# teshnizi/GraphEnvs

Measured on AMD Instinct MI355X. Metric: env-steps/sec (whole node), ShortestPath-v0 n=64 m=192 batch=65536, 1/2/4/8 GPU, higher is better.
Workload: dtype u64; 1 GPU; ShortestPath-v0 n_nodes=64 n_edges=192 weighted, 65536 env slots per GPU, random valid actions on device, same-step autoreset (seed-exact G(n,m)+features on device); envs_per_gpu=65536, prefetch_period=0, episodes_finished_per_gpu=6165512, settle_steps=128, parallelism=batch shard x1, no collective

## Files before the change

### graphenvs_amd/csrc/ge_api.hip

```cpp
#include <math.h>
#include <stdio.h>
#include <stdlib.h>
#include <string.h>

#include <initializer_list>
#include <memory>
#include <new>
#include <vector>

#include "ge_params.h"
#include "ge_platform.h"
#include "ge_reset.h"
#include "ge_features.h"
#include "ge_step.h"
#include "ge_tsp_eval.h"
#include "ge_spare.h"

#define GE_MAX_BUCKETS 4
struct GeBucket {
  bool used;
  bool list_only;
  struct { int lds, pre, grid; } graph;
  struct { int lds, pre_off, threads, grid; } gen;
};
struct GePlan {
  int n_buckets;
  GeBucket bk[GE_MAX_BUCKETS];
  int nseed;
  bool feat_fast;
  int f64_lds, f64_pre_off, feat_grid;
  GeLds inject;
};
static int bucket_of(int n) { return n <= 128 ? 0 : (n <= 256 ? 1 : (n <= 512 ? 2 : 3)); }
static bool takes_generic(const GeParams &C) { return C.n > 64 || C.spatial; }

typedef void (*GeBaselineFn)(GeParams, GeRagged, int, uint8_t *, uint64_t);
struct GeKernels {
  void (*reset)(GeParams, GeRagged, const uint32_t *, GeRun, GeInject, int, int);
  void (*features)(GeParams, GeRagged, GeRun, int, int);
  void (*features64)(GeParams, GeRagged, GeRun, int);
  void (*feat_combine)(GeParams, GeRagged, GeRun);
  void (*swap)(GeParams, GeRagged, GeRagged, ge_buffers, int);
  void (*sample)(GeParams, GeRagged, uint64_t, int64_t *);
  void (*dc_range)(GeParams, GeRagged, const int64_t *);
  void (*tsp_closure)(GeParams, GeRagged, int, uint8_t *, uint64_t, int);
  GeBaselineFn tsp_tour, mis_baseline, steiner_baseline;
  void (*step[2])(GeParams, GeRagged, const int64_t *, uint64_t);
  int step_threads;
  size_t step_lds;
  bool step_quad;
  void (*step_path64[2][2])(GeParams, const int64_t *, uint64_t);
};

struct ge_engine {
  GeParams P;
  ge_config cfg;
  GeKernels k = {};
  GePlan plan = {};
  hipEvent_t ev[4];
  bool have_events = false;
  int n_classes = 0;
  GeRagged R = {};
  int aw_max;
  std::vector<GeParams> classes;
  bool loaded = false;
  bool seeded = false;
  bool streams = false;
  bool spares = false;
  GeParams PS;
  GeRagged RS = {};
  std::vector<GeParams> classesS;
  int period = 0, swap_parts = 1;
  int64_t pending_calls = 0;
  int32_t *refill_list = nullptr, *refill_count = nullptr;
};

static GeRun run_full() { GeRun r = {GE_ITEMS_ALL, 1, 0, 0, 0, 0, 0}; return r; }
static GeRun run_inject(bool seeds) { GeRun r = {GE_ITEMS_ALL, seeds ? 2 : 0, 0, 0, 1, 0, 0}; return r; }
static GeRun run_continue() { GeRun r = {GE_ITEMS_ALL, 0, 1, 1, 0, 0, 0}; return r; }
static GeRun run_queue(const ge_engine *e) { GeRun r = {GE_ITEMS_QUEUE, 0, 1, 0, 0, 0, e->spares ? 2 : GE_SEED_DEPTH}; return r; }
static GeRun run_refill() { GeRun r = {GE_ITEMS_QUEUE, 0, 1, 0, 0, 1, 2}; return r; }
static GeRun as_list(GeRun r) { r.items = GE_ITEMS_LIST; return r; }


static thread_local char g_err[256] = "";
static int fail(int code, const char *msg) { snprintf(g_err, sizeof(g_err), "%s", msg); return code; }
extern "C" const char *ge_last_error(void) { return g_err; }
extern "C" int ge_abi_version(void) { return GE_ABI_VERSION; }
#ifndef GE_SOURCE_HASH
#define GE_SOURCE_HASH "unknown"
#endif
static const char g_source_hash[] = "GE_SOURCE_HASH=" GE_SOURCE_HASH;
extern "C" const char *ge_source_hash(void) { return g_source_hash + 15; }

static const int kMaxLds = 160 * 1024;
static const GeInject kNoInject = {nullptr, nullptr, nullptr, nullptr, nullptr};
static int step_blocks(int64_t B) { return (int)((B + GE_STEP_BLOCK - 1) / GE_STEP_BLOCK); }
static int prefix_bytes(int64_t B) { return (step_blocks(B) + 2) * 4; }
static bool carves_fit(std::initializer_list<int> bytes) { for (int b : bytes) if (b > kMaxLds) return false; return true; }
static int resident_grid(int lds, int64_t B) {
  int per_cu = kMaxLds / (lds > 0 ? lds : 1);
  if (per_cu > 16) per_cu = 16;
  if (per_cu < 1) per_cu = 1;
  return 256 * per_cu > B ? (int)B : 256 * per_cu;
}
static int64_t obs_len(const GeParams &P) { return (int64_t)P.n * P.F + (int64_t)P.E * P.Fe + 2 * (int64_t)P.E; }
static bool prunes(const GeParams &P) { return (P.env_type == GE_LONGEST_PATH || P.env_type == GE_TSP) && P.parenting >= 2; }
#ifndef GE_NP_EARLY_MAX
#define GE_NP_EARLY_MAX 256
#endif

#define GE_FOR_ENV(env_type, stmt)                                                           \
  do {                                                                                       \
// ... 144 lines not shown
  k.sample = ge_k_sample<RAGGED>;
  k.dc_range = ge_k_dc_range<RAGGED>;
  k.tsp_closure = ge_k_tsp_closure<RAGGED>;
  k.tsp_tour = ge_k_tsp_tour<RAGGED>;
  k.mis_baseline = ge_k_mis_baseline<RAGGED>;
  k.steiner_baseline = ge_k_steiner_baseline<RAGGED>;
  k.step[0] = ge_k_step<ENV, false, RAGGED, 0>; k.step[1] = ge_k_step<ENV, true, RAGGED, 0>;
  k.step_threads = GE_STEP_BLOCK;
  k.step_lds = (size_t)GE_STEP_BLOCK * e->P.W * 8 + GE_STEP_BLOCK + 64;
  if constexpr (ENV == GE_STEINER_TREE || ENV == GE_MULTICAST_ROUTING) {
    if (edge_quad(e)) {
      k.step[0] = ge_k_step_edge<ENV, false, RAGGED>; k.step[1] = ge_k_step_edge<ENV, true, RAGGED>;
      k.step_quad = true;
      k.step_threads = GE_EDGE_THREADS;
      k.step_lds = ge_edge_lds_bytes(e->aw_max, e->P.W) + (RAGGED ? GE_EDGE_CLASS_BYTES : 0);
    }
  }
  if constexpr (ENV == GE_LONGEST_PATH || ENV == GE_TSP) {
    if (prunes(e->P) && e->P.W > GE_MAXW) { k.step[0] = ge_k_step<ENV, false, RAGGED, 2>; k.step[1] = ge_k_step<ENV, true, RAGGED, 2>; }
    else if (prunes(e->P)) { k.step[0] = ge_k_step<ENV, false, RAGGED, 1>; k.step[1] = ge_k_step<ENV, true, RAGGED, 1>; }
  }
  if constexpr (!RAGGED) {
    if (path64(e)) {
      k.step_path64[0][0] = ge_k_step_path64<false, false>; k.step_path64[0][1] = ge_k_step_path64<false, true>;
      k.step_path64[1][0] = ge_k_step_path64<true, false>; k.step_path64[1][1] = ge_k_step_path64<true, true>;
    }
  }
}

static bool raise_lds(const void *kernel, size_t bytes) {
  (void)kernel;
  return bytes <= 64 * 1024 || (hipError_t)GE_SET_MAX_DYN_LDS(kernel, bytes) == hipSuccess;
}

static int finish_create(ge_engine *e) {
  const GeParams &P = e->P;
  const bool rg = e->n_classes > 0;
  const int nblk = step_blocks(P.B), pre2 = prefix_bytes(P.B);
  GE_FOR_ENV(P.env_type, if (rg) (select_kernels<ENV, true>(e)); else (select_kernels<ENV, false>(e)));
  GePlan &L = e->plan;
  auto behind = [&](int body, int &pre) { pre = ge_align16(body); return pre + pre2; };
  const GeParams *first = rg ? e->classes.data() : &e->P;
  const int n_classes = rg ? e->n_classes : 1;
  L.n_buckets = rg ? GE_MAX_BUCKETS : 1;
  int graph_lds = 0, gen_lds = 0;
  int gen_body = 0, f64_body = 0;
  for (int b = 0; b < L.n_buckets; b++) {
    GeBucket &K = L.bk[b];
    int graph = 0, gen = 0, all = 0, waves = 1;
    for (const GeParams *C = first; C < first + n_classes; C++) {
      if (C->bucket != b) continue;
      K.used = true;
      if (C->lds.total > graph) graph = C->lds.total;
      if (C->ldsf.total > all) all = C->ldsf.total;
      if (takes_generic(*C)) { if (C->ldsf.total > gen) gen = C->ldsf.total; if (C->ldsf.waves > waves) waves = C->ldsf.waves; }
      else { L.feat_fast = true; const int body = ge_f64_pre_off(C->E, C->env_type == GE_TSP, nblk); if (body > f64_body) f64_body = body; }
    }
    if (!K.used) continue;
    K.list_only = gen == 0;
    if (gen > gen_body) gen_body = gen;
    K.graph.grid = resident_grid(graph, P.B);
    K.graph.pre = P.lds.pre; K.graph.lds = graph;
    if (rg && P.lds.pre != 0) K.graph.lds = behind(graph, K.graph.pre);
    if (K.graph.lds > graph_lds) graph_lds = K.graph.lds;
    K.gen.threads = GE_WAVE * waves;
    K.gen.pre_off = P.ldsf.pre; K.gen.lds = P.ldsf.total;
    if (rg) K.gen.lds = behind(K.list_only ? all : gen, K.gen.pre_off);
    K.gen.grid = resident_grid(K.gen.lds, P.B);
    if (K.list_only && (rg || K.gen.grid > 8)) K.gen.grid = 8;
    if (K.gen.lds > gen_lds) gen_lds = K.gen.lds;
  }
  if (!rg) L.inject = inject_carve(P, P.B);
  if (!carves_fit({graph_lds, L.inject.total, gen_lds})) return fail(GE_E_TOOBIG, "per-env graph does not fit 160 KiB of LDS");
  L.nseed = (resident_grid(graph_lds, P.B) + 63) / 64;
  if (!raise_lds((const void *)e->k.reset, graph_lds > L.inject.total ? graph_lds : L.inject.total)) return fail(GE_E_LAUNCH, "cannot raise the dynamic LDS limit of the reset kernel");
  if (!raise_lds((const void *)e->k.step[0], e->k.step_lds) || !raise_lds((const void *)e->k.step[1], e->k.step_lds))
    return fail(GE_E_LAUNCH, e->k.step_quad ? "cannot raise the dynamic LDS limit of the edge step kernel" : "cannot raise the dynamic LDS limit of the step kernel");
  L.f64_pre_off = ge_align16(f64_body);
  L.f64_lds = L.feat_fast ? L.f64_pre_off + GE_F64_ITEMS * 4 * 4 + 16 : 0;
  if (!carves_fit({L.f64_lds})) return fail(GE_E_TOOBIG, "feature kernel does not fit LDS");
  if (!raise_lds((const void *)e->k.features, gen_lds)) return fail(GE_E_LAUNCH, "cannot raise the dynamic LDS limit of the feature kernel");
  if (L.feat_fast && !raise_lds((const void *)e->k.features64, L.f64_lds)) return fail(GE_E_LAUNCH, "cannot raise the dynamic LDS limit of the n<=64 feature kernel");
  L.feat_grid = resident_grid(L.feat_fast ? L.f64_lds : gen_body, P.B);
  return GE_OK;
}

extern "C" int ge_create(const ge_config *cfg, const ge_buffers *bufs, ge_engine **out) {
  if (!bufs || !out) return fail(GE_E_BADARG, "null argument");
  GeParams P;
  int rc = derive(cfg, P);
  if (rc != GE_OK) return rc;
  rc = check_buffers(P, bufs);
  if (rc != GE_OK) return rc;
  P.buf = *bufs;
  std::unique_ptr<ge_engine> e(new (std::nothrow) ge_engine());
  if (!e) return fail(GE_E_BADARG, "out of host memory");
  e->P = P; e->cfg = *cfg; e->aw_max = P.AW;
  rc = finish_create(e.get());
  if (rc == GE_OK) *out = e.release();
  return rc;
}

extern "C" int64_t ge_ragged_table_bytes(int32_t n_classes) { return (int64_t)sizeof(GeParams) * (n_classes > 0 ? n_classes : 0); }

extern "C" int ge_create_ragged(const ge_config *cfgs, const ge_buffers *bufs, int32_t n_classes, void *class_table,
                                int32_t *slot_class, int32_t *class_start, ge_engine **out) {
  if (!cfgs || !bufs || !out || !class_table || !slot_class || !class_start || n_classes < 1) return fail(GE_E_BADARG, "null argument");
  const int t = cfgs[0].env_type;
  int64_t total = 0;
  for (int c = 0; c < n_classes; c++) total += cfgs[c].num_envs;
  if (total > 8192 * GE_STEP_BLOCK) return fail(GE_E_TOOBIG, "num_envs > 2M per engine");
  std::unique_ptr<ge_engine> e(new (std::nothrow) ge_engine());
  if (!e) return fail(GE_E_BADARG, "out of host memory");
  e->classes.resize(n_classes);
  std::vector<int32_t> start(n_classes + 1, 0), cls_of((size_t)total);
  int widest = 0, aw_max = 0;
  for (int c = 0; c < n_classes; c++) {
    GeParams &C = e->classes[c];
    int rc = derive(&cfgs[c], C, (int)total);
    if (rc == GE_OK) rc = check_buffers(C, &bufs[c]);
    if (rc == GE_OK && (cfgs[c].env_type != t || cfgs[c].autoreset != cfgs[0].autoreset || cfgs[c].seed_stride != cfgs[0].seed_stride))
      rc = fail(GE_E_BADARG, "the classes of a multi-class engine share env_type, autoreset and seed_stride");
    if (rc == GE_OK && (cfgs[c].weighted != cfgs[0].weighted || cfgs[c].parenting != cfgs[0].parenting || cfgs[c].spatial != cfgs[0].spatial ||
                        cfgs[c].is_eval_env != cfgs[0].is_eval_env))
      rc = fail(GE_E_BADARG, "the classes of a multi-class engine share weighted, parenting, spatial and is_eval_env (they differ in n, m and the per-instance scalars only)");
    if (rc == GE_OK && (cfgs[c].env_index_base != cfgs[0].env_index_base + start[c] || bufs[c].seed != bufs[0].seed + start[c] ||
                        bufs[c].episode != bufs[0].episode + start[c] || bufs[c].mt_state != bufs[0].mt_state + (int64_t)start[c] * GE_SEED_DEPTH * 2 * GE_MT_N))
      rc = fail(GE_E_BADARG, "classes follow one another in slot order: env_index_base, seed, episode and mt_state of class c start at its first global slot");
    if (rc == GE_OK && (bufs[c].reset_list != bufs[0].reset_list || bufs[c].reset_count != bufs[0].reset_count || bufs[c].work_list != bufs[0].work_list ||
                        bufs[c].work_count != bufs[0].work_count || bufs[c].slot_rec != bufs[0].slot_rec + 2 * (int64_t)start[c]))
      rc = fail(GE_E_BADARG, "reset_list, reset_count, work_list and work_count are engine-wide (the same pointers in every class), and slot_rec of class c starts at its first global slot");
    if (rc != GE_OK) return rc;
    C.buf = bufs[c];
    start[c + 1] = start[c] + cfgs[c].num_envs;
    for (int i = start[c]; i < start[c + 1]; i++) cls_of[(size_t)i] = c;
    if (C.n > e->classes[widest].n) widest = c;
    if (C.AW > aw_max) aw_max = C.AW;
  }
  if (prunes(e->classes[widest]) && e->classes[widest].W > GE_MAXW)
    for (int c = 0; c < n_classes; c++)
      if (!bufs[c].prune_scratch) return fail(GE_E_BADARG, "parenting >= 2 with a class above 512 nodes runs the residual-graph walks in memory for every class: each class needs prune_scratch ([B_c, 4, W_c] uint64)");
  for (int b = 0; b < GE_MAX_BUCKETS; b++) {
    for (int pass = 0; pass < 2; pass++) {
      int gen_lds = 0;
      for (GeParams &C : e->classes) if (bucket_of(C.n) == b) {
        C.bucket = b;
        if (pass == 0) ge_make_ldsf(C, (int)total); else ge_make_ldsf(C, (int)total, 0, 160 * 1024 - 2048);
        ge_tune_feat_parts(C);
        if (takes_generic(C) && C.ldsf.total > gen_lds) gen_lds = C.ldsf.total;
      }
      if (2 * (gen_lds + prefix_bytes(total)) <= kMaxLds) break;
    }
  }
  e->P = e->classes[widest];
  e->P.B = (int32_t)total;
  for (const GeParams &C : e->classes) if (C.feat_parts > e->P.feat_parts) e->P.feat_parts = C.feat_parts;
  e->P.buf = bufs[0];
  e->P.env_index_base = cfgs[0].env_index_base;
  e->cfg = cfgs[0]; e->cfg.num_envs = (int32_t)total;
  e->n_classes = n_classes;
  e->aw_max = aw_max;
  e->P.AW = aw_max;
  if (hipMemcpy(class_table, e->classes.data(), sizeof(GeParams) * (size_t)n_classes, hipMemcpyHostToDevice) != hipSuccess ||
      hipMemcpy(slot_class, cls_of.data(), sizeof(int32_t) * (size_t)total, hipMemcpyHostToDevice) != hipSuccess ||
      hipMemcpy(class_start, start.data(), sizeof(int32_t) * (size_t)(n_classes + 1), hipMemcpyHostToDevice) != hipSuccess) {
    return fail(GE_E_LAUNCH, "cannot copy the class table to the device");
// ... 40 lines not shown
  if (e->n_classes > 0 && !class_table_spare) return fail(GE_E_BADARG, "a multi-class engine needs class_table_spare (ge_ragged_table_bytes)");
  int rc = GE_OK;
  if (e->n_classes == 0) rc = check_image(e->P, sp[0].image);
  for (int c = 0; c < e->n_classes && rc == GE_OK; c++) rc = check_image(e->classes[c], sp[c].image);
  if (rc != GE_OK) return rc;
  e->refill_list = sp[0].refill_list; e->refill_count = sp[0].refill_count;
  e->PS = image_view(e->P, sp[0].image, e->refill_list, e->refill_count);
  if (e->n_classes > 0) {
    e->classesS.resize(e->n_classes);
    for (int c = 0; c < e->n_classes; c++) e->classesS[c] = image_view(e->classes[c], sp[c].image, e->refill_list, e->refill_count);
    if (hipMemcpy(class_table_spare, e->classesS.data(), sizeof(GeParams) * (size_t)e->n_classes, hipMemcpyHostToDevice) != hipSuccess)
      return fail(GE_E_LAUNCH, "cannot copy the spare class table to the device");
    e->RS = e->R; e->RS.classes = (const GeParams *)class_table_spare;
  }
  e->P.spare_state = sp[0].state; e->P.swap_list = sp[0].swap_list; e->P.swap_count = sp[0].swap_count;
  e->PS.spare_state = sp[0].state;
  e->period = sp[0].period; e->pending_calls = 0;
  const GeParams &P = e->P;
  const int64_t slot_bytes = (int64_t)P.n * P.F * 4 + (int64_t)P.E * (16 + 4 * P.Fe + 2 + 1 + (P.buf.rev_edge ? 4 : 0)) + (int64_t)P.n * P.W * 8 * (P.buf.range_bits ? 2 : 1) + P.A;
  int parts = (int)(slot_bytes / 8192); if (parts < 1) parts = 1; if (parts > 16) parts = 16;
  if (parts >= 4) parts = GE_SWAP_GROUPS;
  e->swap_parts = parts;
  e->spares = true;
  return GE_OK;
}

extern "C" int ge_destroy(ge_engine *e) {
  if (!e) return GE_OK;
  if (e->have_events) for (int k = 0; k < 4; k++) (void)hipEventDestroy(e->ev[k]);
  delete e;
  return GE_OK;
}

static int check_launch(const char *what) {
  static const bool debug_sync = getenv("GE_DEBUG_SYNC") != nullptr;
  if (debug_sync) {
    fprintf(stderr, "[graphenvs] %s ...\n", what); fflush(stderr);
    const hipError_t hs = hipDeviceSynchronize();
    fprintf(stderr, "[graphenvs] %s %s\n", what, hs == hipSuccess ? "done" : hipGetErrorString(hs)); fflush(stderr);
    if (hs != hipSuccess) { snprintf(g_err, sizeof(g_err), "%s: %s (GE_DEBUG_SYNC)", what, hipGetErrorString(hs)); return GE_E_LAUNCH; }
  }
  hipError_t hr = hipGetLastError();
  if (hr != hipSuccess) { snprintf(g_err, sizeof(g_err), "%s: %s", what, hipGetErrorString(hr)); return GE_E_LAUNCH; }
  return GE_OK;
}

static int launch_seed(ge_engine *e, const uint32_t *seeds, int jlo, void *stream) {
  const int64_t items = (int64_t)(GE_SEED_DEPTH - jlo) * e->P.B;
  int64_t grid = (items + GE_WAVE - 1) / GE_WAVE;
  if (grid > 8192) grid = 8192;
  GE_LAUNCH(ge_k_seed, (int)grid, 2 * GE_WAVE, GE_SEED_LDS_BYTES, stream, e->P, seeds, jlo);
  return check_launch("seed kernel");
}

static int launch_combine(ge_engine *e, const GeParams &V, const GeRagged &VR, GeRun run, bool small, void *stream) {
  int64_t items = (int64_t)(run.items == GE_ITEMS_ALL ? V.B : (small ? 64 : 4096)) * V.n;
  int grid = (int)((items + 255) / 256); if (grid > 8192) grid = 8192;
  GE_LAUNCH(e->k.feat_combine, grid, 256, prefix_bytes(V.B), stream, V, VR, run);
  return check_launch("feature combine kernel");
}

static int spread(int grid, int B, bool queue) { return queue ? grid : (B < grid * 4 ? B : grid * 4); }

static int fast_grid(const ge_engine *e, int B, bool queue, bool small) {
  const int g = spread(e->plan.feat_grid, B, queue);
  return small && g > 64 ? 64 : g;
}

static int generic_grid(const ge_engine *e, const GeBucket &K, const GeParams &V, GeRun run, bool small) {
  const bool queue = run.items == GE_ITEMS_QUEUE, list = e->plan.feat_fast;
  if (K.list_only) return K.gen.grid;
  int64_t want = list ? (int64_t)K.gen.grid * (queue ? 1 : 4) : fast_grid(e, V.B, queue, small);
  want *= ge_feat_workgroups(V.feat_parts);
  if (!list && queue && !run.refill && want > 4608) want = 4608;
  if (small && want > 288) want = 288;
  return want > 65535 * 16 ? 65535 * 16 : (int)want;
}

static int launch_features(ge_engine *e, const GeParams &V, const GeRagged &VR, GeRun run, bool small, void *stream) {
  const GePlan &L = e->plan;
  const GeRun rest = L.feat_fast ? as_list(run) : run;
  int rc = GE_OK;
  if (L.feat_fast) {
    GE_LAUNCH(e->k.features64, fast_grid(e, V.B, run.items == GE_ITEMS_QUEUE, small), GE_F64_THREADS, L.f64_lds, stream, V, VR, run, L.f64_pre_off);
    rc = check_launch("feature kernel (n <= 64)");
  }
  for (int b = 0; b < L.n_buckets && rc == GE_OK; b++) {
    const GeBucket &K = L.bk[b];
    if (!K.used) continue;
    GE_LAUNCH(e->k.features, generic_grid(e, K, V, run, small), K.gen.threads, K.gen.lds, stream, V, VR, rest, K.gen.pre_off, e->n_classes > 0 ? b : -1);
    rc = check_launch(L.feat_fast ? "feature kernel (fallback list)" : "feature kernel");
  }
  if (rc != GE_OK || V.feat_parts == 1) return rc;
  return launch_combine(e, V, VR, rest, small, stream);
}

static int launch_seq_baseline(ge_engine *e, const GeParams &P, const GeRagged &VR, int queue, void *stream) {
  const uint64_t slot_bytes = e->n_classes > 0 ? 0 : eval_slot_bytes(P);
  const int pre = prefix_bytes(P.B);
  int g = (P.B + GE_TSP_EVAL_THREADS - 1) / GE_TSP_EVAL_THREADS; if (g > 4096) g = 4096;
  if (P.env_type == GE_MAX_INDEPENDENT_SET) {
    GE_LAUNCH(e->k.mis_baseline, g, GE_TSP_EVAL_THREADS, pre, stream, P, VR, queue, (uint8_t *)P.buf.eval_scratch, slot_bytes);
    return check_launch("MaxIndependentSet baseline kernel");
  }
  if (P.env_type == GE_STEINER_TREE) {
    GE_LAUNCH(e->k.steiner_baseline, g, GE_TSP_EVAL_THREADS, pre, stream, P, VR, queue, (uint8_t *)P.buf.eval_scratch, slot_bytes);
    return check_launch("SteinerTree baseline kernel");
  }
  const int pre_off = GE_WAVE * P.W * 8;
  GE_LAUNCH(e->k.tsp_closure, P.B < 2048 ? P.B : 2048, GE_TSP_EVAL_THREADS, pre_off + pre, stream, P, VR, queue, (uint8_t *)P.buf.eval_scratch, slot_bytes, pre_off);
  int rc = check_launch("TSP baseline: closure kernel");
  if (rc != GE_OK) return rc;
  GE_LAUNCH(e->k.tsp_tour, g, GE_TSP_EVAL_THREADS, pre, stream, P, VR, queue, (uint8_t *)P.buf.eval_scratch, slot_bytes);
  return check_launch("TSP baseline: tour kernel");
}

static int launch_reset(ge_engine *e, const GeParams &V, const GeRagged &VR, const uint32_t *seeds, GeRun run, const GeInject &inj, bool small, void *stream) {
  int rc = GE_OK;
  const bool queue = run.items == GE_ITEMS_QUEUE;
  if (run.restart == 1) rc = launch_seed(e, seeds, 0, stream);
  else if (run.restart == 2) rc = launch_seed(e, inj.seeds, 1, stream);
  if (rc != GE_OK) return rc;
  if (run.cont) {
    int64_t g = ((int64_t)V.B + GE_WAVE - 1) / GE_WAVE; if (g > 8192) g = 8192;
    GE_LAUNCH(ge_k_seed_next, (int)g, 2 * GE_WAVE, GE_SEED_LDS_BYTES, stream, V);
    rc = check_launch("seed kernel (next ring entry)");
    if (rc != GE_OK) return rc;
  }
  const GePlan &L = e->plan;
  int nseed = queue ? L.nseed : 0;
  if (small && nseed > 2) nseed = 2;
  GeParams V2 = V;
  if (run.inject) { V2.nocolw = 0; V2.nowsort = 0; }
  for (int b = 0; b < L.n_buckets && rc == GE_OK; b++) {
    const GeBucket &K = L.bk[b];
    if (!K.used) continue;
    int g = spread(K.graph.grid, V.B, queue), lds = K.graph.lds;
    if (small && g > 128) g = 128;
    V2.lds.pre = K.graph.pre;
    if (run.inject) { V2.lds = L.inject; lds = L.inject.total; }
    GE_LAUNCH(e->k.reset, g + nseed, GE_RESET_THREADS, lds, stream, V2, VR, seeds, run, inj, nseed, e->n_classes > 0 ? b : -1);
    rc = check_launch("reset kernel");
    nseed = 0;
  }
  if (rc != GE_OK) return rc;
  bool baseline = eval_slot_bytes(V) != 0;
  for (const GeParams &C : e->classes) baseline = baseline || eval_slot_bytes(C) != 0;
  if (!run.inject && baseline) rc = launch_seq_baseline(e, V, VR, queue ? 1 : 0, stream);
  if (rc != GE_OK) return rc;
  if (!run.inject) rc = launch_features(e, V, VR, run, small, stream);
  if (rc == GE_OK && run.restart) e->seeded = true;
  if (rc == GE_OK && run.restart == 1 && e->P.buf.stream_state) e->streams = true;
  return rc;
}

static int refill_spares(ge_engine *e, void *stream) {
  GE_LAUNCH(ge_k_refill_list, step_blocks(e->P.B), GE_STEP_BLOCK, 64, stream, e->P, e->refill_list, e->refill_count);
  int rc = check_launch("refill list kernel");
  if (rc != GE_OK) return rc;
  e->pending_calls = 0;
  return launch_reset(e, e->PS, e->RS, nullptr, run_refill(), kNoInject, false, stream);
}
static int invalidate_spares(ge_engine *e, void *stream) {
  if (!e->spares) return GE_OK;
  if (hipMemsetAsync(e->P.spare_state, 0, (size_t)e->P.B, (hipStream_t)stream) != hipSuccess) return fail(GE_E_LAUNCH, "hipMemsetAsync failed");
  return (e->seeded && e->P.autoreset) ? refill_spares(e, stream) : GE_OK;
}

static int clear_queue(ge_engine *e, void *stream) {
  const size_t bytes = sizeof(int32_t) * (size_t)step_blocks(e->P.B);
  if (hipMemsetAsync(e->P.buf.reset_count, 0, bytes, (hipStream_t)stream) != hipSuccess) return fail(GE_E_LAUNCH, "hipMemsetAsync failed");
  if (e->spares && hipMemsetAsync(e->P.swap_count, 0, bytes, (hipStream_t)stream) != hipSuccess) return fail(GE_E_LAUNCH, "hipMemsetAsync failed");
  return GE_OK;
}

extern "C" int ge_reset(ge_engine *e, const uint32_t *seeds, void *stream) {
  if (!e || !seeds) return fail(GE_E_BADARG, "null argument");
  int rc = clear_queue(e, stream);
  if (rc != GE_OK) return rc;
  rc = launch_reset(e, e->P, e->R, seeds, run_full(), kNoInject, false, stream);
  if (rc == GE_OK) e->loaded = true;
  if (rc == GE_OK) rc = invalidate_spares(e, stream);
  return rc;
}

extern "C" int ge_reset_continue(ge_engine *e, void *stream) {
  if (!e) return fail(GE_E_BADARG, "null argument");
  if (e->n_classes > 0) return fail(GE_E_UNSUPPORTED, "ge_reset_continue is not built for the multi-class engine");
  if (e->spares) return fail(GE_E_UNSUPPORTED, "ge_reset_continue on an engine with spares: an image generated ahead of time would leave the streams of the wrong episode behind");
  if (!e->P.buf.stream_state) return fail(GE_E_STATE, "ge_reset_continue needs ge_buffers.stream_state (the streams every reset leaves behind)");
  if (!e->loaded || !e->seeded || !e->streams) return fail(GE_E_STATE, "ge_reset_continue before ge_reset: there is no stream to continue");
  int rc = clear_queue(e, stream);
  if (rc != GE_OK) return rc;
  return launch_reset(e, e->P, e->R, nullptr, run_continue(), kNoInject, false, stream);
}

extern "C" int ge_inject_state(ge_engine *e, const int64_t *links, const uint8_t *wcode, const float *x,
                               const int32_t *terminals, const uint32_t *seeds, void *stream) {
  if (!e || !links || !wcode || !x) return fail(GE_E_BADARG, "null argument");
  if (e->n_classes > 0) return fail(GE_E_UNSUPPORTED, "ge_inject_state is not built for the multi-class engine (inject into uniform engines)");
  const int t = e->P.env_type;
  if ((t == GE_SHORTEST_PATH || t == GE_LONGEST_PATH || t == GE_STEINER_TREE || t == GE_MULTICAST_ROUTING || t == GE_DISTRIBUTION_CENTER ||
       t == GE_PERISHABLE_DELIVERY) && !terminals)
    return fail(GE_E_BADARG, "terminals required (source / destinations, targets, or pickups then drop-offs)");
  if (!seeds && e->P.autoreset && !e->seeded)
    return fail(GE_E_STATE, "ge_inject_state without seeds on an engine with autoreset whose generator states were never seeded: pass seeds, or call ge_reset first");
  GeInject inj = {links, wcode, x, terminals, seeds};
  int rc = clear_queue(e, stream);
  if (rc != GE_OK) return rc;
  rc = launch_reset(e, e->P, e->R, nullptr, run_inject(seeds != nullptr), inj, false, stream);
  if (rc == GE_OK) e->loaded = true;
  if (rc == GE_OK) rc = invalidate_spares(e, stream);
  return rc;
}

extern "C" int ge_sample_actions(ge_engine *e, uint64_t policy_seed, int64_t *actions, void *stream);

static void launch_step(ge_engine *e, bool sample, const int64_t *actions, uint64_t policy_seed, void *stream) {
  const GeKernels &k = e->k;
  const int grid = step_blocks(e->P.B);
  if (path64(e)) GE_LAUNCH(k.step_path64[sample][e->spares], grid, k.step_threads, k.step_lds, stream, e->P, actions, policy_seed);
  else GE_LAUNCH(k.step[sample], grid, k.step_threads, k.step_lds, stream, e->P, e->R, actions, policy_seed);
}

static bool dc_range(const ge_engine *e) {
  if (e->P.env_type != GE_DISTRIBUTION_CENTER) return false;
  if (e->n_classes == 0) return e->P.n <= 64;
  for (const GeParams &C : e->classes) if (C.n <= 64) return true;
  return false;
}

static int check_state(const ge_engine *e) {
  if (!e->loaded) return fail(GE_E_STATE, "the engine holds no episode yet: call ge_reset (or ge_inject_state) first");
  if (e->P.autoreset && !e->seeded) return fail(GE_E_STATE, "autoreset needs seeded generator states: call ge_reset, or ge_inject_state with seeds");
  return GE_OK;
}

extern "C" int ge_step_only(ge_engine *e, const int64_t *actions, void *stream) {
  if (!e || !actions) return fail(GE_E_BADARG, "null argument");
  int rc = check_state(e);
  if (rc != GE_OK) return rc;
  if (dc_range(e)) {
    const int rows = e->n_classes > 0 ? 64 : e->P.n;
    GE_LAUNCH(e->k.dc_range, (e->P.B + GE_WAVE - 1) / GE_WAVE, GE_WAVE, (size_t)rows * GE_WAVE * 8 + GE_WAVE * 64, stream, e->P, e->R, actions);
    rc = check_launch("coverage range kernel");
    if (rc != GE_OK) return rc;
  }
  launch_step(e, false, actions, 0, stream);
  return check_launch("step kernel");
}

static int sample_and_step(ge_engine *e, uint64_t policy_seed, int64_t *scratch, void *stream) {
  int rc = check_state(e);
  if (rc != GE_OK) return rc;
// ... 163 lines not shown
```

### graphenvs_amd/csrc/ge_features.h

```cpp
#pragma once
#include "ge_params.h"
#include "ge_platform.h"
#include "ge_reset.h"

struct GeFctx {
  uint64_t *abits; int *rowptr; uint16_t *scw;
  uint64_t *quads; uint32_t *rq; int zq;
  uint8_t *c8;
  double *sigma, *delta, *coeff, *bcw;
  double *bcw0; int wave_f64;
  double *bc, *clos;
  double *prx, *prn, *sinv, *diff, *diff2, *clus;
  uint8_t *mark;
  uint16_t *ord, *lvl;
};

GE_DEV GeFctx ge_carve_f(const GeParams &P, int tid) {
  unsigned char *s = ge_dyn_smem();
  const GeLdsF &L = P.ldsf;
  const int n = P.n, an = ((n * 8 + 15) & ~15) / 8;
  GeFctx c;
  c.rowptr = (int *)(s + L.rowptr); c.quads = (uint64_t *)(s + L.colw); c.c8 = (uint8_t *)(s + L.colw); c.rq = (uint32_t *)(s + L.rq); c.zq = L.zq;
  c.bc = (double *)(s + L.bc); c.clos = (double *)(s + L.clos);
  unsigned char *w = s + L.wave0 + (tid >> 6) * L.wave_stride;
// ... 567 lines not shown
  }
  if (live) {
    float *xr = G.x + (nbase + lane) * F + P.nflag;
    xr[0] = (float)(2.0 * (double)deg); xr[3] = (float)x; xr[4] = (float)clus;
  }
  ge_wave_sync();
}


GE_DEV int ge_slot_class(const GeRagged &R, int env) { return (int)ge_uniform_u32((uint32_t)R.slot_class[env]); }

#ifndef GE_GEN_WPS
#define GE_GEN_WPS 0
#endif
#if GE_GEN_WPS > 0
#define GE_GEN_KERNEL GE_KERNEL_LB(512, GE_GEN_WPS)
#else
#define GE_GEN_KERNEL GE_KERNEL
#endif
template <bool RAGGED>
GE_GEN_KERNEL ge_k_features(GeParams P, GeRagged R, GeRun run, int pre_off, int bucket) {
  int *pre = (int *)(ge_dyn_smem() + pre_off);
  const bool queue = run.items == GE_ITEMS_QUEUE, list = run.items == GE_ITEMS_LIST;
  if (list) ge_wave_priority(GE_PRIO_PROBE);
  int count = list ? P.buf.work_count[0] : P.B;
  if (list && count > 0) ge_wave_priority(0);
  if (queue) {
    if (ge_tid() < GE_WAVE) ge_queue_prefix_wave(P, pre, ge_tid());
    ge_sync();
    count = pre[(P.B + GE_STEP_BLOCK - 1) / GE_STEP_BLOCK];
  }
  const int fparts = (list && !RAGGED) ? 1 : P.feat_parts;
  const int nparts = ge_feat_workgroups(fparts);
  for (int q = ge_bid(); q < count * nparts; q += ge_gdim()) {
    const int item = q / nparts, part = q % nparts;
    const int env = queue ? ge_queue_slot(P, pre, item) : (list ? P.buf.work_list[item] : item);
    if constexpr (RAGGED) {
      const int cls = ge_slot_class(R, env);
      const GeParams &C = R.classes[cls];
      if (bucket >= 0 && C.bucket != bucket) continue;
      if (queue && part == 0 && ge_tid() == 0) ge_finish_item(P, run, env);
      if (part < ge_feat_workgroups(C.feat_parts)) ge_features_generic_env(C, env - R.class_start[cls], part, C.feat_parts);
    } else {
      if (queue && part == 0 && ge_tid() == 0) ge_finish_item(P, run, env);
      ge_features_generic_env(P, env, part, fparts);
    }
  }
}

template <bool RAGGED>
GE_KERNEL ge_k_feat_combine(GeParams P, GeRagged R, GeRun run) {
  int *pre = (int *)ge_dyn_smem();
  const bool queue = run.items == GE_ITEMS_QUEUE, list = run.items == GE_ITEMS_LIST;
  int count = list ? P.buf.work_count[0] : P.B;
  if (queue) {
    if (ge_tid() < GE_WAVE) ge_queue_prefix_wave(P, pre, ge_tid());
    ge_sync();
    count = pre[(P.B + GE_STEP_BLOCK - 1) / GE_STEP_BLOCK];
  }
  const int nmax = P.n;
  for (int64_t g = (int64_t)ge_bid() * ge_bdim() + ge_tid(); g < (int64_t)count * nmax; g += (int64_t)ge_gdim() * ge_bdim()) {
    const int item = (int)(g / nmax), v = (int)(g % nmax);
    int env = queue ? ge_queue_slot(P, pre, item) : (list ? P.buf.work_list[item] : item);
    int cls = 0;
    if constexpr (RAGGED) { cls = R.slot_class[env]; env -= R.class_start[cls]; }
    const GeParams &C = RAGGED ? R.classes[cls] : P;
    const int n = C.n, nparts = C.feat_parts;
    if (v >= n || nparts == 1) continue;
    double acc = 0.0;
    for (int p = 0; p < nparts; p++) acc += C.buf.feat_scratch[((int64_t)env * nparts + p) * n + v];
    if (n > 2) acc *= 1.0 / (double)((int64_t)(n - 1) * (int64_t)(n - 2));
    C.buf.x[((int64_t)env * n + v) * C.F + C.nflag + 1] = (float)acc;
  }
}

#ifndef GE_F64_WPS
#define GE_F64_WPS 6
#endif
#if GE_F64_WPS > 0
#define GE_F64_KERNEL GE_KERNEL_LB(GE_F64_THREADS, GE_F64_WPS)
#else
#define GE_F64_KERNEL GE_KERNEL
#endif
template <bool RAGGED>
GE_F64_KERNEL ge_k_features64(GeParams P, GeRagged R, GeRun run, int tail_off) {
  const int nblk = (P.B + GE_STEP_BLOCK - 1) / GE_STEP_BLOCK;
  int *const pre = (int *)ge_dyn_smem();
  int *const items = (int *)(ge_dyn_smem() + tail_off);
  int *const ovf_flag = items + GE_F64_ITEMS * 4;
  const bool queue = run.items == GE_ITEMS_QUEUE;
  int count = P.B;
  for (int base = 0;; base += GE_F64_ITEMS) {
    const int tid = ge_tid_fresh();
    if (queue) {
      if (tid < GE_WAVE) ge_queue_prefix_wave(P, pre, tid);
      ge_sync();
      count = pre[nblk];
    }
    const int total = count + (count + 3) / 4;
    if (ge_bid() + (int64_t)base * ge_gdim() >= total) break;
    if (tid < GE_F64_ITEMS * 4) {
      const int64_t q = ge_bid() + (int64_t)(base + (tid >> 2)) * ge_gdim();
      const int sub = tid & 3;
      int qi = -1;
      if (q < count) qi = sub == 0 ? (int)q : -1;
      else if (q < total) { const int64_t k = 4 * (q - count) + sub; qi = k < count ? (int)k : -1; }
      items[tid] = qi < 0 ? -1 : (queue ? ge_queue_slot(P, pre, qi) : qi);
    }
    ge_sync();
    for (int i = 0; i < GE_F64_ITEMS; i++) {
      const int64_t q = ge_bid() + (int64_t)(base + i) * ge_gdim();
      if (q >= total) break;
      if (q < count) {
        const int env = items[4 * i];
        if (queue && ge_tid() == 0) ge_finish_item(P, run, env);
        if constexpr (RAGGED) {
          const int cls = ge_slot_class(R, env);
          const GeParams &C = R.classes[cls];
          if (C.n > 64) {
            if (ge_tid() == 0) { int k = atomicAdd(&P.buf.work_count[0], 1); P.buf.work_list[k] = env; }
            continue;
          }
          ge_f64_walk_env(C, env - R.class_start[cls], ovf_flag, P.buf.work_count, P.buf.work_list, env);
        } else {
          ge_f64_walk_env(P, env, ovf_flag, P.buf.work_count, P.buf.work_list, env);
        }
      } else {
        const int t2 = ge_tid_fresh();
        const int wv = t2 >> 6, lane = t2 & (GE_WAVE - 1);
        const int env = items[4 * i + wv];
        if (env >= 0) {
          if constexpr (RAGGED) {
            const int cls = ge_slot_class(R, env);
            const GeParams &C = R.classes[cls];
            if (C.n <= 64) ge_f64_node_env(C, env - R.class_start[cls], ge_dyn_smem() + wv * ge_f64_node_wave_bytes(R.f64_tsp_e, C.env_type == GE_TSP), lane);
          } else {
            ge_f64_node_env(P, env, ge_dyn_smem() + wv * ge_f64_node_wave_bytes(P.E, P.env_type == GE_TSP), lane);
          }
        }
        ge_sync();
      }
    }
    ge_sync();
  }
}
```

### graphenvs_amd/csrc/ge_params.h

```cpp
#pragma once
#include <stdint.h>

#include "../../include/graphenvs.h"

#define GE_WAVE 64
#define GE_MT_N 624
#define GE_MT_M 397
#ifndef GE_DC_LANES
#define GE_DC_LANES 16
#endif
#ifndef GE_STEP_BLOCK
#define GE_STEP_BLOCK 256
#endif
#define GE_RESET_THREADS 128
#define GE_SEED_TILE_STRIDE 68
#define GE_SEED_LDS_BYTES (2 * 16 * GE_SEED_TILE_STRIDE * 4 + 64 * 4 + 64)
#ifndef GE_RESET_WAVES_PER_SIMD
#define GE_RESET_WAVES_PER_SIMD 6
#endif

struct GeLds {
  int mt;
  int mt2;
  int wm;
  int abits;
  int elist;
  int fill;
  int rowptr;
  int colw;
  int wsort;
  int tmp;
  int dist;
  int perm;
  int f64a;
  int bits;
  int misc;
  int fw;
  int dcs;
  int kou;
  int pre;
  int total;
};

struct GeLdsF {
  int rowptr, colw, bc, clos;
  int rq;
  int zq;
  int wave0, wave_stride, waves;
  int w_sigma, w_mark, w_ord, w_lvl;
  int node, abits, scw, prx, clus;
  int wl;
  int pre, total;
};

struct GeParams {
  int32_t env_type, B, n, m, E, W, F, Fe, A, AW, T, ng, nflag;
  int32_t weighted, parenting, n_dests, is_eval, autoreset, complete;
  int32_t spatial;
  int32_t feat_parts;
  int32_t np_early;
  int32_t nocolw;
  int32_t nowsort;
  int32_t cost_off;
  uint64_t div_m;
  double n_choices;
  double max_distance;
  double dt_min, dt_max;
  int64_t env_index_base, seed_stride, node_id_base, edge_row_stride;
  ge_buffers buf;
  GeLds lds;
  GeLdsF ldsf;
  uint8_t *spare_state;
  int32_t *swap_list, *swap_count;
  int32_t bucket;
};

enum { GE_ITEMS_ALL = 0, GE_ITEMS_QUEUE = 1, GE_ITEMS_LIST = 2 };
struct GeRun {
  int32_t items;
  int32_t restart;
  int32_t next;
  int32_t cont;
  int32_t inject;
  int32_t refill;
  int32_t seed_ahead;
};

struct GeRagged {
  const GeParams *classes;
  const int32_t *slot_class;
  const int32_t *class_start;
  int32_t n_classes;
  int32_t f64_tsp_e;
};

static inline int ge_align16(int v) { return (v + 15) & ~15; }

static inline void ge_make_lds(GeParams &P, int queue_B) {
  GeLds &L = P.lds;
  int o = 0;
  auto take = [&](int bytes) { int r = o; o = ge_align16(o + bytes); return r; };
  L.mt = take(GE_MT_N * 4);
  L.mt2 = take(GE_MT_N * 4);
  {
    const bool matrix_env = P.env_type == GE_SHORTEST_PATH || P.env_type == GE_LONGEST_PATH || P.env_type == GE_STEINER_TREE ||
                            P.env_type == GE_MULTICAST_ROUTING || P.env_type == GE_DISTRIBUTION_CENTER || P.env_type == GE_PERISHABLE_DELIVERY;
    const int matrix = (P.np_early && matrix_env && P.weighted) ? ((P.n * P.n + 7) / 8) * 4 : 0;
    int nb = matrix > 16 ? matrix : 16; if (P.m > nb) nb = P.m; if (P.n > nb) nb = P.n;
    if (P.spatial && 32 * P.n > nb) nb = 32 * P.n;
    P.cost_off = 0;
    if (P.env_type == GE_DISTRIBUTION_CENTER) { P.cost_off = matrix; if (P.cost_off + P.n > nb) nb = P.cost_off + P.n; }
    L.wm = take(nb); }
  L.abits = take(P.n * P.W * 8);
  L.elist = take((P.complete ? P.n : (P.m > 0 ? P.m : 1)) * 4);
  L.fill = take(P.n * 4);
  L.rowptr = take((P.n + 1) * 4);
  L.colw = take((P.nocolw ? 8 : (P.E > 0 ? P.E : 1)) * 2);
  L.wsort = take(P.nowsort ? 16 : (P.E > 0 ? P.E : 1));
  L.tmp = take(P.complete ? 16 : (P.E > 0 ? P.E : 1) * 4);
  L.dist = take(P.n * 4);
  L.perm = take(P.n * 4);
  {
    const bool dist_env = P.env_type == GE_MULTICAST_ROUTING || P.env_type == GE_DISTRIBUTION_CENTER || P.env_type == GE_PERISHABLE_DELIVERY;
    int need = (P.is_eval || dist_env) ? 2 * P.n * 8 : 0, mw = ((P.E > P.n ? P.E : P.n) / 64 + 2) * 8; L.f64a = take(need > mw ? need : mw); }
  L.bits = take(6 * P.W * 8);
  L.misc = take(16 * 4);
  L.fw = (P.env_type == GE_PERISHABLE_DELIVERY && P.n <= 128) ? take(P.n * P.n * 8) : 0;
  L.dcs = (P.env_type == GE_DISTRIBUTION_CENTER && P.n <= 64) ? take(P.n * GE_DC_LANES * 8 + 64 * GE_DC_LANES) : 0;
  L.kou = (P.env_type == GE_STEINER_TREE && P.is_eval && P.n_dests > 1 && P.n_dests < P.n - 1) ? take(2 * P.n * P.W * 8 + P.T * 16) : 0;
  { int pb = ((queue_B + GE_STEP_BLOCK - 1) / GE_STEP_BLOCK + 1) * 4; L.pre = L.mt; if (pb > GE_MT_N * 8) { L.pre = take(pb); } }
  if (o < GE_SEED_LDS_BYTES) o = GE_SEED_LDS_BYTES;
  L.total = o;
}

#ifndef GE_FEAT_SRC_PER_WAVE
#define GE_FEAT_SRC_PER_WAVE 4
#endif
static inline void ge_tune_feat_parts(GeParams &P) {
  if (P.feat_parts <= 1) return;
  int want = P.n / (P.ldsf.waves * GE_FEAT_SRC_PER_WAVE);
  if (want < 2) want = 2;
  if (want < P.feat_parts) P.feat_parts = want;
}

#ifndef GE_BCW_REG_W
#define GE_BCW_REG_W 8
#endif
static inline void ge_make_ldsf(GeParams &P, int queue_B, int force_waves = 0, int budget = 160 * 1024 / 2) {
  GeLdsF &L = P.ldsf;
  int o = 0;
  auto take = [&](int bytes) { int r = o; o = ge_align16(o + bytes); return r; };
  const int n = P.n, E = P.E > 0 ? P.E : 1;
  const bool split = P.feat_parts > 1;
  L.rowptr = take((n + 1) * 4);
  const bool closed = P.complete && P.ng == n;
  const int nquads = (E + 3 * n) / 4 + 1;
  L.zq = nquads - 1;
  L.colw = take(closed ? E : nquads * 8);
  L.rq = closed ? L.colw : take(n * 4);
  L.bc = take(n * 8);
  L.clos = take(n * 8);
  const int common = o;
  L.w_sigma = 0;
  L.w_mark = (P.W <= GE_BCW_REG_W ? 3 : 4) * n * 8 + 8;
  L.w_ord = ge_align16(L.w_mark + n + 1);
  L.w_lvl = L.w_ord + ge_align16(2 * n);
  L.wave_stride = ge_align16(L.w_lvl + 2 * (n + 2));
  const int node_bytes = ge_align16(n * P.W * 8) + (closed ? 0 : ge_align16(E * 2)) + 6 * ge_align16(n * 8);
// ... 36 lines not shown
```

### graphenvs_amd/csrc/ge_platform.h

```cpp
#pragma once
#ifdef GE_EMU
#include "hip_emu.h"
#else
#include <hip/hip_runtime.h>
#include <stdint.h>

#define GE_DEV static __device__ __forceinline__
#define GE_DEVFN __device__
#define GE_KERNEL __global__ void
#define GE_KERNEL_LB(threads, waves_per_simd) __global__ void __launch_bounds__(threads, waves_per_simd)
#define GE_HOSTDEV __host__ __device__ inline
#define GE_CONSTANT static __constant__ const

GE_DEV int ge_tid() { return (int)threadIdx.x; }
GE_DEV int ge_tid_fresh() { int t = (int)threadIdx.x; asm volatile("" : "+v"(t)); return t; }
GE_DEV int ge_bid() { return (int)blockIdx.x; }
GE_DEV int ge_bdim() { return (int)blockDim.x; }
GE_DEV int ge_gdim() { return (int)gridDim.x; }
GE_DEV unsigned char *ge_dyn_smem() {
  extern __shared__ __align__(16) unsigned char ge_smem_raw[];
  return ge_smem_raw;
}
GE_DEV void ge_sync() { __syncthreads(); }
GE_DEV void ge_wave_priority(int p) {
  switch (p) {
    case 0: __builtin_amdgcn_s_setprio(0); break;
    case 1: __builtin_amdgcn_s_setprio(1); break;
    case 2: __builtin_amdgcn_s_setprio(2); break;
    default: __builtin_amdgcn_s_setprio(3); break;
  }
}
GE_DEV void ge_wave_sync() { __builtin_amdgcn_fence(__ATOMIC_SEQ_CST, "workgroup"); __builtin_amdgcn_wave_barrier(); }
GE_DEV void ge_quad_sync() { __builtin_amdgcn_fence(__ATOMIC_SEQ_CST, "wavefront"); }
GE_DEV uint32_t ge_quad_xor1(uint32_t v) { return (uint32_t)__builtin_amdgcn_mov_dpp((int)v, 0xB1, 0xf, 0xf, true); }
GE_DEV uint32_t ge_quad_xor2(uint32_t v) { return (uint32_t)__builtin_amdgcn_mov_dpp((int)v, 0x4E, 0xf, 0xf, true); }
GE_DEV uint64_t ge_quad_gather16(uint32_t v) {
  const uint32_t b0 = (uint32_t)__builtin_amdgcn_mov_dpp((int)v, 0x00, 0xf, 0xf, true), b1 = (uint32_t)__builtin_amdgcn_mov_dpp((int)v, 0x55, 0xf, 0xf, true);
  const uint32_t b2 = (uint32_t)__builtin_amdgcn_mov_dpp((int)v, 0xAA, 0xf, 0xf, true), b3 = (uint32_t)__builtin_amdgcn_mov_dpp((int)v, 0xFF, 0xf, 0xf, true);
  return (uint64_t)((b0 & 0xffffu) | (b1 << 16)) | ((uint64_t)((b2 & 0xffffu) | (b3 << 16)) << 32);
}
GE_DEV uint32_t ge_oct_or32(uint32_t v) {
  v |= (uint32_t)__builtin_amdgcn_mov_dpp((int)v, 0xB1, 0xf, 0xf, true);
  v |= (uint32_t)__builtin_amdgcn_mov_dpp((int)v, 0x4E, 0xf, 0xf, true);
  v |= (uint32_t)__builtin_amdgcn_mov_dpp((int)v, 0x141, 0xf, 0xf, true);
  return v;
}
GE_DEV void ge_lds_add_u32(uint32_t *p, uint32_t v) { atomicAdd(p, v); }
GE_DEV void ge_lds_add_f64(double *p, double v) { unsafeAtomicAdd(p, v); }
GE_DEV void ge_wait_loads() { __builtin_amdgcn_s_waitcnt(0x0F70); }
GE_DEV uint64_t ge_ballot(bool p) { return (uint64_t)__ballot(p ? 1 : 0); }
GE_DEV int ge_shfl_i32(int v, int src) { return __shfl(v, src, 64); }
GE_DEV uint32_t ge_shfl_u32(uint32_t v, int src) { return (uint32_t)__shfl((int)v, src, 64); }
GE_DEV uint64_t ge_shfl_u64(uint64_t v, int src) {
  int lo = __shfl((int)(uint32_t)v, src, 64), hi = __shfl((int)(uint32_t)(v >> 32), src, 64);
  return ((uint64_t)(uint32_t)hi << 32) | (uint32_t)lo;
}
GE_DEV double ge_shfl_f64(double v, int src) { return __longlong_as_double((long long)ge_shfl_u64((uint64_t)__double_as_longlong(v), src)); }
GE_DEV uint32_t ge_readlane_u32(uint32_t v, int idx) { return (uint32_t)__builtin_amdgcn_readlane((int)v, idx); }
GE_DEV uint32_t ge_writelane_u32(uint32_t v, uint32_t val, int idx) { return ((int)(threadIdx.x & 63u) == idx) ? val : v; }
GE_DEV uint32_t ge_uniform_u32(uint32_t v) { return (uint32_t)__builtin_amdgcn_readfirstlane((int)v); }
GE_DEV double ge_u64_as_f64(uint64_t v) { return __longlong_as_double((long long)v); }
GE_DEV uint64_t ge_f64_as_u64(double v) { return (uint64_t)__double_as_longlong(v); }
GE_DEV int ge_popc64(uint64_t v) { return __popcll(v); }
GE_DEV int ge_mbcnt(uint64_t m) { return (int)__builtin_amdgcn_mbcnt_hi((uint32_t)(m >> 32), __builtin_amdgcn_mbcnt_lo((uint32_t)m, 0u)); }
GE_DEV int ge_ctz64(uint64_t v) { return v ? (int)__builtin_ctzll(v) : 64; }
GE_DEV int ge_clz32(uint32_t v) { return v ? (int)__builtin_clz(v) : 32; }

#define GE_LAUNCH(kernel, grid, block, smem, stream, ...) \
  hipLaunchKernelGGL(kernel, dim3((unsigned)(grid)), dim3((unsigned)(block)), (size_t)(smem), (hipStream_t)(stream), __VA_ARGS__)
#define GE_SET_MAX_DYN_LDS(kernel, bytes) \
  hipFuncSetAttribute((const void *)(kernel), hipFuncAttributeMaxDynamicSharedMemorySize, (int)(bytes))
#endif

#define GE_PRIO_STEP 3
#define GE_PRIO_PROBE 3
```

Baseline: 403.4 million env-steps/s.

## Drain fallback feature list inside last block of n<=64 feature kernel

Instead of launching a separate generic feature kernel for the fallback work list after the n<=64 feature kernel, the last workgroup to finish (detected via a device-scope atomic counter with release/acquire fences) processes the list itself. This removes a kernel launch and its dependency gap per step. In exchange, the drain runs serially in one workgroup, which could be slow if the list is long, and it needs an extra memset to reset the counter plus a noinline cold function that reads the kernel arguments through the kernarg pointer.

```diff
diff --git a/graphenvs_amd/csrc/ge_api.hip b/graphenvs_amd/csrc/ge_api.hip
--- a/graphenvs_amd/csrc/ge_api.hip
+++ b/graphenvs_amd/csrc/ge_api.hip
@@ -29,6 +29,7 @@
   int nseed;
   bool feat_fast;
   int f64_lds, f64_pre_off, feat_grid;
+  bool drain;
   GeLds inject;
 };
 static int bucket_of(int n) { return n <= 128 ? 0 : (n <= 256 ? 1 : (n <= 512 ? 2 : 3)); }
@@ -339,6 +340,7 @@
   if (!raise_lds((const void *)e->k.features, gen_lds)) return fail(GE_E_LAUNCH, "cannot raise the dynamic LDS limit of the feature kernel");
   if (L.feat_fast && !raise_lds((const void *)e->k.features64, L.f64_lds)) return fail(GE_E_LAUNCH, "cannot raise the dynamic LDS limit of the n<=64 feature kernel");
   L.feat_grid = resident_grid(L.feat_fast ? L.f64_lds : gen_body, P.B);
+  L.drain = !rg && L.feat_fast && L.bk[0].list_only && P.ldsf.pre <= L.f64_lds;
   return GE_OK;
 }
 
@@ -545,8 +547,11 @@
   const GeRun rest = L.feat_fast ? as_list(run) : run;
   int rc = GE_OK;
   if (L.feat_fast) {
-    GE_LAUNCH(e->k.features64, fast_grid(e, V.B, run.items == GE_ITEMS_QUEUE, small), GE_F64_THREADS, L.f64_lds, stream, V, VR, run, L.f64_pre_off);
+    GeRun fast = run;
+    fast.drain = L.drain ? 1 : 0;
+    GE_LAUNCH(e->k.features64, fast_grid(e, V.B, run.items == GE_ITEMS_QUEUE, small), GE_F64_THREADS, L.f64_lds, stream, V, VR, fast, L.f64_pre_off);
     rc = check_launch("feature kernel (n <= 64)");
+    if (L.drain) return rc;
   }
   for (int b = 0; b < L.n_buckets && rc == GE_OK; b++) {
     const GeBucket &K = L.bk[b];
@@ -633,6 +638,7 @@
 static int clear_queue(ge_engine *e, void *stream) {
   const size_t bytes = sizeof(int32_t) * (size_t)step_blocks(e->P.B);
   if (hipMemsetAsync(e->P.buf.reset_count, 0, bytes, (hipStream_t)stream) != hipSuccess) return fail(GE_E_LAUNCH, "hipMemsetAsync failed");
+  if (e->plan.drain && hipMemsetAsync(e->P.buf.work_count + 2, 0, sizeof(int32_t), (hipStream_t)stream) != hipSuccess) return fail(GE_E_LAUNCH, "hipMemsetAsync failed");
   if (e->spares && hipMemsetAsync(e->P.swap_count, 0, bytes, (hipStream_t)stream) != hipSuccess) return fail(GE_E_LAUNCH, "hipMemsetAsync failed");
   return GE_OK;
 }
diff --git a/graphenvs_amd/csrc/ge_features.h b/graphenvs_amd/csrc/ge_features.h
--- a/graphenvs_amd/csrc/ge_features.h
+++ b/graphenvs_amd/csrc/ge_features.h
@@ -673,6 +673,14 @@
 #else
 #define GE_F64_KERNEL GE_KERNEL
 #endif
+GE_DEV_COLD void ge_f64_drain_list(const GeParams *P0) {
+  const GeParams &P = ge_kernarg0(P0);
+  ge_acquire_device();
+  if (ge_tid() == 0) ge_store_device_i32(&P.buf.work_count[2], 0);
+  const int count = ge_load_device_i32(&P.buf.work_count[0]);
+  for (int k = 0; k < count; k++) ge_features_generic_env(P, ge_load_device_i32(&P.buf.work_list[k]), 0, 1);
+}
+
 template <bool RAGGED>
 GE_F64_KERNEL ge_k_features64(GeParams P, GeRagged R, GeRun run, int tail_off) {
   const int nblk = (P.B + GE_STEP_BLOCK - 1) / GE_STEP_BLOCK;
@@ -734,4 +742,13 @@
     }
     ge_sync();
   }
-}
+  if constexpr (!RAGGED) {
+    if (run.drain) {
+      ge_release_device();
+      ge_sync();
+      if (ge_tid() == 0) items[0] = atomicAdd(&P.buf.work_count[2], 1);
+      ge_sync();
+      if (items[0] == ge_gdim() - 1) ge_f64_drain_list(ge_cold_arg(P));
+    }
+  }
+}
diff --git a/graphenvs_amd/csrc/ge_params.h b/graphenvs_amd/csrc/ge_params.h
--- a/graphenvs_amd/csrc/ge_params.h
+++ b/graphenvs_amd/csrc/ge_params.h
@@ -84,6 +84,7 @@
   int32_t inject;
   int32_t refill;
   int32_t seed_ahead;
+  int32_t drain;
 };
 
 struct GeRagged {
diff --git a/graphenvs_amd/csrc/ge_platform.h b/graphenvs_amd/csrc/ge_platform.h
--- a/graphenvs_amd/csrc/ge_platform.h
+++ b/graphenvs_amd/csrc/ge_platform.h
@@ -1,12 +1,20 @@
 #pragma once
 #ifdef GE_EMU
 #include "hip_emu.h"
+#define GE_DEV_COLD static inline
+GE_DEV void ge_release_device() {}
+GE_DEV void ge_acquire_device() {}
+GE_DEV int32_t ge_load_device_i32(const int32_t *p) { return *(const volatile int32_t *)p; }
+GE_DEV void ge_store_device_i32(int32_t *p, int32_t v) { *(volatile int32_t *)p = v; }
+template <class T> GE_DEV const T *ge_cold_arg(const T &a) { return &a; }
+template <class T> GE_DEV const T &ge_kernarg0(const T *a) { return *a; }
 #else
 #include <hip/hip_runtime.h>
 #include <stdint.h>
 
 #define GE_DEV static __device__ __forceinline__
 #define GE_DEVFN __device__
+#define GE_DEV_COLD static __device__ __attribute__((noinline))
 #define GE_KERNEL __global__ void
 #define GE_KERNEL_LB(threads, waves_per_simd) __global__ void __launch_bounds__(threads, waves_per_simd)
 #define GE_HOSTDEV __host__ __device__ inline
@@ -22,6 +30,19 @@
   return ge_smem_raw;
 }
 GE_DEV void ge_sync() { __syncthreads(); }
+GE_DEV void ge_release_device() { __builtin_amdgcn_fence(__ATOMIC_RELEASE, "agent"); }
+GE_DEV void ge_acquire_device() { __builtin_amdgcn_fence(__ATOMIC_ACQUIRE, "agent"); }
+GE_DEV int32_t ge_load_device_i32(const int32_t *p) { return __hip_atomic_load(p, __ATOMIC_RELAXED, __HIP_MEMORY_SCOPE_AGENT); }
+GE_DEV void ge_store_device_i32(int32_t *p, int32_t v) { __hip_atomic_store(p, v, __ATOMIC_RELAXED, __HIP_MEMORY_SCOPE_AGENT); }
+template <class T> GE_DEV const T *ge_cold_arg(const T &) {
+  return (const T *)(const __attribute__((address_space(4))) void *)__builtin_amdgcn_kernarg_segment_ptr();
+}
+template <class T> GE_DEV const T &ge_kernarg0(const T *a) {
+  const uint64_t v = (uint64_t)a;
+  const uint64_t u = (uint64_t)(uint32_t)__builtin_amdgcn_readfirstlane((int)(uint32_t)v) |
+                     ((uint64_t)(uint32_t)__builtin_amdgcn_readfirstlane((int)(uint32_t)(v >> 32)) << 32);
+  return *(const T *)(const __attribute__((address_space(4))) T *)u;
+}
 GE_DEV void ge_wave_priority(int p) {
   switch (p) {
     case 0: __builtin_amdgcn_s_setprio(0); break;
```

Result: slower. 158.3 million env-steps/s (-60.8%).
